# naver/dust3r

Hardware: NVIDIA H100
Metric: image-pairs/sec (512x384, ViT-L/B+DPT) (higher is better)
Workload: dtype bf16

## Files before the change

dust3r_b200/_lib.py:

```python
from __future__ import annotations

import ctypes as C
import os

from ._lib_fwd import Model

_HERE = os.path.dirname(os.path.abspath(__file__))
LIB_PATH = os.path.join(_HERE, 'libdust3r_b200.so')

_lib = None


class D3RError(RuntimeError):
    pass


class AlignDesc(C.Structure):
    _fields_ = [
        ('n_imgs', C.c_int32), ('n_edges', C.c_int32), ('n_entries', C.c_int32), ('n_chunks', C.c_int32),
        ('max_deg', C.c_int32), ('max_chunks', C.c_int32), ('chunk_px', C.c_int32), ('dist_l2', C.c_int32), ('norm_pw_scale', C.c_int32),
        ('tied_focal', C.c_int32), ('eval_only', C.c_int32),
        ('base_scale', C.c_float), ('pw_break', C.c_float), ('focal_break', C.c_float), ('adam_eps', C.c_float),
        ('beta1', C.c_float), ('beta2', C.c_float),
        ('img_hw', C.c_void_p), ('img_pix_off', C.c_void_p), ('img_ent_ptr', C.c_void_p),
# ... 44 lines not shown
    'd3r_align_small_step': (i32, [_DESC, i32, vp]),
    'd3r_align_reduce_block': (i32, [i32, i32, C.POINTER(i64), C.POINTER(i64)]),
    'd3r_align_loss_grad': (i32, [_DESC, vp, vp, vp, vp]),
    'd3r_align_overflow_flag': (i32, [_DESC, C.POINTER(i32), vp]),
    'd3r_align_pts3d': (i32, [_DESC, vp, vp]),
    'd3r_align_set_debug': (i32, [vp]),
    'd3r_sizeof_pack_entry': (i32, []),
    'd3r_align_stream_slots_per_item': (i32, []),
    'd3r_align_stream_warps_per_cta': (i32, []),
    'd3r_align_stream_max_window': (i32, []),
    'd3r_align_pack_entries': (i32, [vp, i32, i32, i32, i32, vp, vp]),
    'd3r_gemm_bf16': (i32, [vp, vp, vp, vp, vp, vp, i32, i32, i32, i64, u32, vp, vp, i32, i32, i32, vp]),
    'd3r_conv3x3_bf16': (i32, [vp, vp, vp, vp, vp, vp, vp, i32, i32, i32, i32, i32, u32, vp]),
    'd3r_attention_hd64': (i32, [vp, i64, vp, i64, vp, i64, vp, i64, i32, i32, i32, i32, f32, vp]),
    'd3r_conv_transpose_bf16': (i32, [vp, vp, vp, vp, i32, i32, i32, i32, i32, i32, vp]),
    'd3r_conv3x3_head_tail': (i32, [vp, vp, vp, vp, vp, vp, vp, i32, i32, i32, i32, i32, f32, f32, vp]),
    'd3r_layernorm_bf16': (i32, [vp, vp, vp, vp, i32, i32, f32, vp]),
    'd3r_upsample2x_bf16': (i32, [vp, vp, i32, i32, i32, i32, i32, i32, vp]),
    'd3r_im2col_3x3_s2_bf16': (i32, [vp, vp, i32, i32, i32, i32, vp]),
    'd3r_patch_im2col16': (i32, [vp, vp, i32, i32, i32, vp]),
    'd3r_linear_head_postprocess': (i32, [vp, vp, vp, i32, i32, i32, i32, i32, i32, f32, f32, vp]),
    'd3r_set_gemm_impl': (None, [i32]),
    'd3r_set_gemm_store': (None, [i32]),
    'd3r_set_conv_store': (None, [i32]),
    'd3r_set_attention_impl': (None, [i32]),
    'd3r_clean_pointcloud': (i32, [i32, vp, vp, i32, vp, vp, vp, vp, vp, f32, f32, vp]),
    'd3r_procrustes_moments': (i32, [i32, i32, vp, vp, vp, vp, vp]),
    'd3r_weiszfeld_focal': (i32, [i32, i32, i32, vp, vp, i32, vp, vp]),
    'd3r_nearest_neighbours': (i32, [i32, i32, vp, vp, vp, vp]),
    'd3r_image_resize_crop_normalize': (i32, [vp, i32, i32, i32, i32, vp, vp, i32, vp, vp, i32, i32, i32, i32, i32, i32, i32,
                                              vp, vp, vp, vp]),
    'd3r_sizeof_jpeg_desc': (i32, []),
    'd3r_jpeg_decode_workspace_bytes': (i64, [_JPEG, i64]),
    'd3r_jpeg_decode': (i32, [_JPEG, vp, i64, vp, vp, vp, i64, vp]),
    'd3r_segment_sky_workspace_bytes': (i64, [i32, i64]),
    'd3r_segment_sky': (i32, [i32, vp, vp, i32, i64, vp, vp, vp, i64, vp]),
    'd3r_nanmedian_workspace_bytes': (i64, [i32]),
    'd3r_segmented_nanmedian': (i32, [i32, i64, vp, vp, vp, i64, vp]),
    'd3r_criterion_workspace_bytes': (i64, [i32, i64, i64, i32]),
    'd3r_criterion': (i32, [i32, i64, i64, i32, i32, f32, f32] + [vp] * 15 + [i64, vp]),
    'd3r_sizeof_model': (i32, []),
    'd3r_encode_workspace_bytes': (i64, [_MODEL, i32, i32, i32]),
    'd3r_encode_images': (i32, [_MODEL, vp, i32, i32, i32, vp, vp, i64, vp]),
    'd3r_decode_workspace_bytes': (i64, [_MODEL, i32, i32, i32, i32, i32]),
    'd3r_decode_pairs': (i32, [_MODEL, vp, i32, i32, i32, vp, i32, i32, i32, C.POINTER(i32), C.POINTER(i32), i32,
                               vp, vp, vp, vp, vp, i64, vp]),
# ... 80 lines not shown
```

dust3r_b200/csrc/gemm_host.cu:

```cuda
#include "gemm_wgmma.cuh"
#include "gemm_host.h"
#include "prof.h"

namespace d3r {
namespace gemm {

static int pick_block_n(int N, int mode, uint32_t flags, int conv_m_tiles = 0) {
  if (flags & F_HEAD_FINAL) return 128;
  if (conv_m_tiles > 0) return (N == 256 && (conv_m_tiles + 1) / 2 >= 4 * (num_sms() / 2)) ? 256 : 128;
  if (N % 256 == 0 && pick_epi(mode, flags) != EPI_GENERIC) return 256;
  if (N % 128 == 0) return 128;
  if (N % 64 == 0) return 64;
  return (N > 128) ? 128 : 64;
}

static int g_impl = 2;
constexpr int kPairMinKb = 4;
static bool use_pair(int bn, int num_kb) { return bn >= 128 && (g_impl == 1 || (g_impl == 2 && num_kb >= kPairMinKb)); }

static int g_store = 1;
static int g_conv_store = 1;

static int grid_for(bool pair, int m_tiles, int n_tiles) {
  if (pair) {
    const int items = ((m_tiles + 1) / 2) * n_tiles;
    const int max_clusters = num_sms() / 2;
    return 2 * (items < max_clusters ? items : max_clusters);
  }
  const int items = m_tiles * n_tiles;
  return items < num_sms() ? items : num_sms();
}

static const char* prof_tag(const Params& p, int bn, bool pair) {
  return (p.mode == 1) ? ((p.flags & F_HEAD_FINAL) ? (pair ? "conv3x3_head_tail_2cta" : "conv3x3_head_tail")
                                                   : (pair ? "conv3x3_wgmma_2cta" : "conv3x3_wgmma"))
                       : (bn == 256 ? (pair ? "gemm_wgmma_2cta_bn256" : "gemm_wgmma_bn256")
                                    : (pair ? "gemm_wgmma_2cta_bn128" : (bn == 128 ? "gemm_wgmma_bn128" : "gemm_wgmma_bn64")));
}

template <int BN, int EPI, bool PAIR, bool TMA_STORE = false>
static int launch(const CUtensorMap& ta, const CUtensorMap& tb, const CUtensorMap& to, const Params& p, int m_tiles, int n_tiles,
                  cudaStream_t st) {
  constexpr int kSmem = Cfg<BN, TMA_STORE>::kSmemBytes;
  static unsigned long long attr_devices = 0;
  if (first_launch_on_this_device(attr_devices))
    D3R_CUDA(cudaFuncSetAttribute(gemm_kernel<BN, EPI, PAIR, TMA_STORE>, cudaFuncAttributeMaxDynamicSharedMemorySize, kSmem));
  const int grid = grid_for(PAIR, m_tiles, n_tiles);
  char detail[96];
  snprintf(detail, sizeof(detail), "M=%d N=%d K=%d flags=0x%x mode=%d epi=%d", p.M, p.N, p.K, (unsigned)p.flags, p.mode, EPI);
  prof::Scope scope(prof_tag(p, BN, PAIR), st, 2.0 * double(p.M) * double(p.N) * double(p.K), 0.0, 1, detail);
  D3R_CUDA(pdl::launch_clustered(gemm_kernel<BN, EPI, PAIR, TMA_STORE>, dim3(grid), dim3(kNumThreads), size_t(kSmem), st, PAIR ? 2 : 1,
                                 ta, tb, to, p));
  D3R_LAUNCH_CHECK();
  return D3R_OK;
}

template <int BN, bool PAIR>
static int launch_conv(const CUtensorMap& ta, const CUtensorMap& tb, const CUtensorMap& to, const ConvMaps& cm, const Params& p,
                       int m_tiles, int n_tiles, cudaStream_t st) {
  constexpr int kSmem = Cfg<BN, true>::kSmemBytes;
  static unsigned long long attr_devices = 0;
  if (first_launch_on_this_device(attr_devices))
    D3R_CUDA(cudaFuncSetAttribute(conv_kernel<BN, PAIR>, cudaFuncAttributeMaxDynamicSharedMemorySize, kSmem));
  const int grid = grid_for(PAIR, m_tiles, n_tiles);
  char detail[96];
  snprintf(detail, sizeof(detail), "M=%d N=%d K=%d flags=0x%x mode=%d epi=%d", p.M, p.N, p.K, (unsigned)p.flags, p.mode, EPI_GENERIC);
  prof::Scope scope(prof_tag(p, BN, PAIR), st, 2.0 * double(p.M) * double(p.N) * double(p.K), 0.0, 1, detail);
  D3R_CUDA(pdl::launch_clustered(conv_kernel<BN, PAIR>, dim3(grid), dim3(kNumThreads), size_t(kSmem), st, PAIR ? 2 : 1, ta, tb, to, cm, p));
  D3R_LAUNCH_CHECK();
  return D3R_OK;
}

template <int BN, bool PAIR>
static int dispatch_epi(int epi, const CUtensorMap& ta, const CUtensorMap& tb, const CUtensorMap* to, const Params& p, int m_tiles,
                        int n_tiles, cudaStream_t st) {
  if constexpr (BN == 256) {
    if (to) {
      switch (epi) {
        case EPI_RESID: return launch<BN, EPI_RESID, PAIR, true>(ta, tb, *to, p, m_tiles, n_tiles, st);
        case EPI_ACT: return launch<BN, EPI_ACT, PAIR, true>(ta, tb, *to, p, m_tiles, n_tiles, st);
        case EPI_ROPE: return launch<BN, EPI_ROPE, PAIR, true>(ta, tb, *to, p, m_tiles, n_tiles, st);
      }
    }
  }
  switch (epi) {
    case EPI_RESID: return launch<BN, EPI_RESID, PAIR>(ta, tb, tb, p, m_tiles, n_tiles, st);
    case EPI_ACT: return launch<BN, EPI_ACT, PAIR>(ta, tb, tb, p, m_tiles, n_tiles, st);
// ... 13 lines not shown
    case 256: return pair ? dispatch_epi<256, true>(epi, ta, tb, to, p, m_tiles, n_tiles, st) : dispatch_epi<256, false>(epi, ta, tb, to, p, m_tiles, n_tiles, st);
    case 128: return pair ? dispatch_epi<128, true>(epi, ta, tb, nullptr, p, m_tiles, n_tiles, st) : dispatch_epi<128, false>(epi, ta, tb, nullptr, p, m_tiles, n_tiles, st);
    case 64: return launch<64, EPI_GENERIC, false>(ta, tb, tb, p, m_tiles, n_tiles, st);
  }
  set_error("unsupported BLOCK_N %d", bn);
  return D3R_ERR_INVALID;
}

static int make_tmap_b(CUtensorMap* m, const void* B, int N, int taps, int Kc, int bn, int num_kb, const char* op) {
  cuuint64_t dims[3] = {(cuuint64_t)Kc, (cuuint64_t)taps, (cuuint64_t)N};
  cuuint64_t str[2] = {(cuuint64_t)Kc * 2, (cuuint64_t)taps * Kc * 2};
  cuuint32_t box[3] = {(cuuint32_t)BLOCK_K, 1, (cuuint32_t)(use_pair(bn, num_kb) ? bn / 2 : bn)};
  return encode_tensor_map(m, B, 3, dims, str, box, op);
}

int gemm_bf16(const void* A, long long lda, const void* B, Params p, cudaStream_t st) {
  D3R_CHECK_ARG(A && B, "gemm: null operand");
  D3R_CHECK_ARG(p.M > 0 && p.N > 0 && p.K > 0, "gemm: bad shape %d %d %d", p.M, p.N, p.K);
  D3R_CHECK_ARG(p.N % 32 == 0, "gemm: N=%d must be a multiple of 32", p.N);
  D3R_CHECK_ARG(p.K % 8 == 0 && lda % 8 == 0, "gemm: K=%d / lda=%lld must be multiples of 8 (16-byte TMA strides)", p.K, lda);
  D3R_CHECK_ARG((reinterpret_cast<uintptr_t>(A) & 15) == 0 && (reinterpret_cast<uintptr_t>(B) & 15) == 0, "gemm: operands must be 16-byte aligned");
  p.mode = 0;
  p.num_kb = (p.K + BLOCK_K - 1) / BLOCK_K;
  const int bn = pick_block_n(p.N, p.mode, p.flags);
  CUtensorMap ta, tb;
  {
    cuuint64_t dims[2] = {(cuuint64_t)p.K, (cuuint64_t)p.M};
    cuuint64_t str[1] = {(cuuint64_t)lda * 2};
    cuuint32_t box[2] = {(cuuint32_t)BLOCK_K, (cuuint32_t)BLOCK_M};
    int rc = encode_tensor_map(&ta, A, 2, dims, str, box, "gemm");
    if (rc) return rc;
  }
  int rc = make_tmap_b(&tb, B, p.N, 1, p.K, bn, p.num_kb, "gemm");
  if (rc) return rc;
  CUtensorMap to;
  const bool f32 = (p.flags & F_RESID_INPLACE) != 0;
  const long long row_bytes = p.ldo * (f32 ? 4 : 2);
  const bool staged = g_store == 1 && bn == 256 && pick_epi(p.mode, p.flags) != EPI_GENERIC && p.ldo >= p.N && row_bytes % 16 == 0 &&
                      (reinterpret_cast<uintptr_t>(p.out) & 15) == 0;
  if (staged) {
    cuuint64_t dims[2] = {(cuuint64_t)p.N, (cuuint64_t)p.M};
    cuuint64_t str[1] = {(cuuint64_t)row_bytes};
    cuuint32_t box[2] = {(cuuint32_t)(f32 ? 32 : 64), 64};
    rc = encode_tensor_map(&to, p.out, 2, dims, str, box, "gemm output", f32 ? CU_TENSOR_MAP_DATA_TYPE_FLOAT32 : CU_TENSOR_MAP_DATA_TYPE_BFLOAT16);
    if (rc) return rc;
  }
  return dispatch(bn, ta, tb, staged ? &to : nullptr, p, (p.M + BLOCK_M - 1) / BLOCK_M, st);
}

static int make_tmap_conv_io(CUtensorMap* m, const void* base, int B, int H, int W, int C, int tile_w, const char* op) {
  const int bw = tile_w < 64 ? tile_w : 64;
  cuuint64_t dims[4] = {(cuuint64_t)C, (cuuint64_t)W, (cuuint64_t)H, (cuuint64_t)B};
  cuuint64_t str[3] = {(cuuint64_t)C * 2, (cuuint64_t)W * C * 2, (cuuint64_t)H * W * C * 2};
  cuuint32_t box[4] = {64, (cuuint32_t)bw, (cuuint32_t)(64 / bw), 1};
  return encode_tensor_map(m, base, 4, dims, str, box, op);
}

static bool aligned16(const void* ptr) { return (reinterpret_cast<uintptr_t>(ptr) & 15) == 0; }

int conv3x3_bf16(const void* x_nhwc, const void* w_packed, int B, int H, int W, int Cin, int Cout, Params p, cudaStream_t st) {
  D3R_CHECK_ARG(x_nhwc && w_packed, "conv3x3: null operand");
  D3R_CHECK_ARG(Cin % 8 == 0 && Cout % 32 == 0, "conv3x3: Cin=%d must be a multiple of 8 and Cout=%d of 32", Cin, Cout);
  p.mode = 1;
  p.M = B * H * W;
  p.N = Cout;
  p.cin_blocks = (Cin + BLOCK_K - 1) / BLOCK_K;
  p.K = 9 * Cin;
  p.num_kb = 9 * p.cin_blocks;
  p.cB = B; p.cH = H; p.cW = W;
  int tw = 16;
// ... 57 lines not shown
                      float* conf, int B, int H, int W, int depth_mode, int conf_mode, float conf_min, float conf_max, cudaStream_t st) {
  D3R_CHECK_ARG(x_nhwc && w_packed && w4 && b4 && pts3d, "conv3x3_head_tail: null buffer");
  D3R_CHECK_ARG(B > 0 && H > 0 && W > 0, "conv3x3_head_tail: bad shape B=%d H=%d W=%d", B, H, W);
  D3R_CHECK_ARG(depth_mode >= 0 && depth_mode <= 2, "conv3x3_head_tail: depth_mode %d out of range", depth_mode);
  D3R_CHECK_ARG(conf_mode >= 0 && conf_mode <= 2, "conv3x3_head_tail: conf_mode %d out of range", conf_mode);
  D3R_CHECK_ARG(conf_mode == 0 || conf, "conv3x3_head_tail: conf_mode %d without a conf buffer", conf_mode);
  Params p{};
  p.flags = F_HEAD_FINAL | (bias ? F_BIAS : 0);
  p.bias = bias;
  p.w4 = w4; p.b4 = b4;
  p.pts3d = pts3d; p.conf = conf;
  p.depth_mode = depth_mode; p.conf_mode = conf_mode;
  p.conf_min = conf_min; p.conf_max = conf_max;
  return conv3x3_bf16(x_nhwc, w_packed, B, H, W, 128, 128, p, st);
}

}
}

using namespace d3r;

extern "C" void d3r_set_gemm_impl(int32_t impl) { gemm::g_impl = impl; }
extern "C" void d3r_set_gemm_store(int32_t store) { gemm::g_store = store; }
extern "C" void d3r_set_conv_store(int32_t store) { gemm::g_conv_store = store; }

extern "C" int d3r_gemm_bf16(const void* A, const void* B, void* out, const float* bias, const void* add0, void* out2,
                             int32_t M, int32_t N, int32_t K, int64_t ldo, uint32_t flags, const float* rope_cos,
                             const float* rope_sin, int32_t rope_cols, int32_t tokens_per_img, int32_t grid_w, void* stream) {
  gemm::Params p{};
  p.M = M; p.N = N; p.K = K;
  p.flags = flags;
  p.out = out; p.out2 = out2; p.add0 = add0; p.bias = bias; p.ldo = ldo;
  p.rope_cos = rope_cos; p.rope_sin = rope_sin; p.rope_cols = rope_cols; p.tokens_per_img = tokens_per_img; p.grid_w = grid_w;
  D3R_CHECK_ARG(!(flags & gemm::F_BIAS) || bias, "gemm: F_BIAS without bias");
  D3R_CHECK_ARG(!(flags & gemm::F_ROPE) || (rope_cos && rope_sin && tokens_per_img > 0 && grid_w > 0), "gemm: F_ROPE without tables");
  D3R_CHECK_ARG(!(flags & (gemm::F_CONVT | gemm::F_HEAD_FINAL)),
                "gemm: F_CONVT / F_HEAD_FINAL have their own entry points, d3r_conv_transpose_bf16 / d3r_conv3x3_head_tail");
  return gemm::gemm_bf16(A, K, B, p, (cudaStream_t)stream);
}

extern "C" int d3r_conv3x3_bf16(const void* x_nhwc, const void* w_packed, void* out, const float* bias, const void* add0,
                                const void* add1, void* out2, int32_t B, int32_t H, int32_t W, int32_t Cin, int32_t Cout,
                                uint32_t flags, void* stream) {
  gemm::Params p{};
  p.flags = flags;
  p.out = out; p.out2 = out2; p.add0 = add0; p.add1 = add1; p.bias = bias;
// ... 16 lines not shown
```

dust3r_b200/csrc/gemm_wgmma.cuh:

```cuda
#pragma once
#include "d3r_common.cuh"
#include "sm90_ptx.cuh"
#include "pdl.cuh"

namespace d3r {
namespace gemm {

constexpr int BLOCK_M = 128;
constexpr int BLOCK_K = 64;
constexpr int WGMMA_K = 16;
constexpr int kNumThreads = 384;
constexpr int kConsumerWarps = 8;

enum : uint32_t {
  F_BIAS = 1u << 0,
  F_GELU = 1u << 1,
  F_RELU = 1u << 2,
  F_OUT_F32 = 1u << 3,
  F_RESID_INPLACE = 1u << 4,
  F_ADD0 = 1u << 5,
  F_ADD1 = 1u << 6,
  F_OUT2_RELU = 1u << 7,
  F_ROPE = 1u << 8,
  F_CONVT = 1u << 9,
// ... 4 lines not shown
struct Params {
  int M, N, K;
  int num_kb;
  int mode;
  uint32_t flags;
  void* out;
  void* out2;
  const void* add0;
  const void* add1;
  const float* bias;
  long long ldo;
  const float* rope_cos;
  const float* rope_sin;
  int rope_cols, tokens_per_img, grid_w;
  int cB, cH, cW, cin_blocks, tile_w, tile_h, tiles_x, tiles_y;
  int tk, th_in, tw_in, tCout;
  const float* w4;
  const float* b4;
  float* pts3d;
  float* conf;
  int depth_mode;
  int conf_mode;
  float conf_min, conf_max;
};

enum : int { EPI_GENERIC = 0, EPI_RESID = 1, EPI_ACT = 2, EPI_ROPE = 3, EPI_CONV = 4 };
template <int EPI> struct EpiMask { static constexpr uint32_t value = 0xFFFFFFFFu; };
template <> struct EpiMask<EPI_RESID> { static constexpr uint32_t value = F_BIAS | F_RESID_INPLACE; };
template <> struct EpiMask<EPI_ACT> { static constexpr uint32_t value = F_BIAS | F_GELU | F_RELU; };
template <> struct EpiMask<EPI_ROPE> { static constexpr uint32_t value = F_BIAS | F_ROPE; };
template <> struct EpiMask<EPI_CONV> { static constexpr uint32_t value = F_BIAS | F_RELU | F_ADD0 | F_ADD1 | F_OUT2_RELU; };

struct ConvMaps {
  CUtensorMap out2, add0, add1;
};

__host__ __device__ inline int pick_epi(int mode, uint32_t flags) {
  if (mode != 0) return EPI_GENERIC;
  if ((flags & ~F_BIAS) == F_RESID_INPLACE) return EPI_RESID;
  if ((flags & ~EpiMask<EPI_ACT>::value) == 0) return EPI_ACT;
  if ((flags & ~EpiMask<EPI_ROPE>::value) == 0) return EPI_ROPE;
  return EPI_GENERIC;
}

template <int BLOCK_N, bool TMA_STORE = false>
struct Cfg {
  static constexpr int kStageA = BLOCK_M * BLOCK_K * 2;
  static constexpr int kStageB = BLOCK_N * BLOCK_K * 2;
  static constexpr int kStages = (BLOCK_N == 256) ? 4 : (BLOCK_N == 128) ? 6 : 8;
  static constexpr int kRing = kStages * (kStageA + kStageB);
  static constexpr int kOutBuf = 64 * 128;
  static constexpr int kStaging = TMA_STORE ? 2 * 2 * kOutBuf : 0;
  static constexpr int kSmemBytes = kRing + kStaging + 1024  + 256  + (TMA_STORE ? 0 : (4 * 128 + 16) * 4) ;
  static_assert(kSmemBytes <= 227 * 1024, "shared memory of one CTA");
};

__device__ __forceinline__ float gelu_erf(float x) {
  constexpr float kU = 0.84932180028801904f;
  constexpr float kP = 0.3275911f * 0.70710678118654752f / kU;
  const float u = fabsf(x) * kU;
  const float t = ptx::rcp_approx(fmaf(kP, u, 1.f));
  float poly = fmaf(0.5f * 1.061405429f, t, 0.5f * -1.453152027f);
  poly = fmaf(poly, t, 0.5f * 1.421413741f);
  poly = fmaf(poly, t, 0.5f * -0.284496736f);
  poly = fmaf(poly, t, 0.5f * 0.254829592f);
  const float e = ptx::ex2_approx(-u * u);
  const float h = x * (poly * t * e);
  return fmaxf(x, 0.f) - fabsf(h);
}

template <int BLOCK_N, int EPI, bool PAIR, bool TMA_STORE>
__device__ __forceinline__ void gemm_body(const CUtensorMap& tmap_a, const CUtensorMap& tmap_b, const CUtensorMap& tmap_o,
                                          const ConvMaps* cm, const Params& p) {
  static_assert(EPI == EPI_CONV ? (TMA_STORE && (BLOCK_N == 256 || BLOCK_N == 128))
                                : (!TMA_STORE || (BLOCK_N == 256 && EPI != EPI_GENERIC)),
                "TMA-store epilogue: specialised projection epilogues on 128x256 tiles, the conv epilogue on 128x256 / 128x128");
  using C = Cfg<BLOCK_N, TMA_STORE>;
  extern __shared__ uint8_t smem_raw[];
  uint8_t* smem = reinterpret_cast<uint8_t*>((reinterpret_cast<uintptr_t>(smem_raw) + 1023) & ~uintptr_t(1023));
  uint8_t* smem_a = smem;
  uint8_t* smem_b = smem + C::kStages * C::kStageA;
  uint8_t* smem_o = smem + C::kRing;
  uint64_t* bars = reinterpret_cast<uint64_t*>(smem + C::kRing + C::kStaging);
  uint64_t* full_bar = bars;
  uint64_t* empty_bar = bars + C::kStages;
  uint64_t* add_bar = bars + 2 * C::kStages;
  float* s_w4 = reinterpret_cast<float*>(reinterpret_cast<uint8_t*>(bars) + 256);

  const int warp = threadIdx.x >> 5, lane = threadIdx.x & 31;
  const uint32_t rank = PAIR ? ptx::cluster_ctarank() : 0u;
  const int n_tiles = (p.N + BLOCK_N - 1) / BLOCK_N;
  const int m_tiles = (p.mode == 1) ? p.cB * p.tiles_y * p.tiles_x : (p.M + BLOCK_M - 1) / BLOCK_M;
  const int m_groups = PAIR ? (m_tiles + 1) / 2 : m_tiles;
  const int total_items = m_groups * n_tiles;
  const int first_item = PAIR ? blockIdx.x / 2 : blockIdx.x;
  const int item_stride = PAIR ? gridDim.x / 2 : gridDim.x;

  if (threadIdx.x == 0) {
    ptx::prefetch_tmap(&tmap_a);
    ptx::prefetch_tmap(&tmap_b);
    if constexpr (TMA_STORE) ptx::prefetch_tmap(&tmap_o);
    for (int s = 0; s < C::kStages; ++s) {
      ptx::mbar_init(ptx::smem_u32(&full_bar[s]), 1);
      ptx::mbar_init(ptx::smem_u32(&empty_bar[s]), (PAIR ? 2 : 1) * kConsumerWarps);
    }
    if constexpr (EPI == EPI_CONV) {
      ptx::prefetch_tmap(&cm->out2);
      ptx::prefetch_tmap(&cm->add0);
      ptx::prefetch_tmap(&cm->add1);
      ptx::mbar_init(ptx::smem_u32(&add_bar[0]), 1);
      ptx::mbar_init(ptx::smem_u32(&add_bar[1]), 1);
    }
    ptx::fence_barrier_init();
  }
  if (!TMA_STORE && (p.flags & F_HEAD_FINAL) && threadIdx.x >= 128) {
    for (int i = threadIdx.x - 128; i < 4 * 128 + 4; i += 256) s_w4[i] = (i < 512) ? p.w4[i] : p.b4[i - 512];
  }
  __syncthreads();
  if constexpr (PAIR) ptx::cluster_sync();
  pdl::sync_with_predecessor();

  if (warp < 4) {
    ptx::setmaxnreg_dec<40>();
    if (warp == 0 && ptx::elect_one()) {
      int stage = 0;
      uint32_t phase = 0;
      for (int item = first_item; item < total_items; item += item_stride) {
        const int tn = item % n_tiles, tm = (item / n_tiles) * (PAIR ? 2 : 1) + int(rank);
        int cb = 0, cy0 = 0, cx0 = 0;
        if (p.mode == 1) {
          cb = tm / (p.tiles_y * p.tiles_x);
          const int r = tm - cb * (p.tiles_y * p.tiles_x);
          cy0 = (r / p.tiles_x) * p.tile_h;
          cx0 = (r % p.tiles_x) * p.tile_w;
        }
        for (int kb = 0; kb < p.num_kb; ++kb) {
          ptx::mbar_wait(ptx::smem_u32(&empty_bar[stage]), phase ^ 1);
          const uint32_t fb = ptx::smem_u32(&full_bar[stage]);
          ptx::mbar_arrive_expect_tx(fb, C::kStageA + C::kStageB);
          const uint32_t sa = ptx::smem_u32(smem_a + stage * C::kStageA);
          const uint32_t sb = ptx::smem_u32(smem_b + stage * C::kStageB);
          int ka, kt = 0;
          if (p.mode == 1) {
            const int tap = kb / p.cin_blocks, cblk = kb - tap * p.cin_blocks;
            const int dy = tap / 3, dx = tap - dy * 3;
            ptx::tma_load_4d(sa, &tmap_a, fb, cblk * BLOCK_K, cx0 + dx - 1, cy0 + dy - 1, cb);
            ka = cblk * BLOCK_K;
            kt = tap;
          } else {
            ptx::tma_load_2d(sa, &tmap_a, fb, kb * BLOCK_K, tm * BLOCK_M);
            ka = kb * BLOCK_K;
          }
          if constexpr (PAIR) {
            constexpr int kHalf = BLOCK_N / 2;
            ptx::tma_load_3d_mc(sb + rank * (kHalf * BLOCK_K * 2), &tmap_b, fb, ka, kt, tn * BLOCK_N + int(rank) * kHalf, 0x3);
          } else {
            ptx::tma_load_3d(sb, &tmap_b, fb, ka, kt, tn * BLOCK_N);
          }
          if (++stage == C::kStages) { stage = 0; phase ^= 1; }
        }
      }
    }
  } else {
    ptx::setmaxnreg_inc<232>();
    const int wg = (threadIdx.x >> 7) - 1;
    const int wq = warp & 3;
    const int q = lane & 3;
    const uint32_t flags = p.flags & EpiMask<EPI>::value;
    constexpr int kNB = BLOCK_N / 8;
    float acc[BLOCK_N / 2];
    int stage = 0;
    uint32_t phase = 0;
    uint32_t out_chunk = 0;
    auto release = [&](int s) {
      if (lane == 0) {
        if constexpr (PAIR) {
          ptx::mbar_arrive_cluster(ptx::smem_u32(&empty_bar[s]), 0);
          ptx::mbar_arrive_cluster(ptx::smem_u32(&empty_bar[s]), 1);
        } else {
          ptx::mbar_arrive(ptx::smem_u32(&empty_bar[s]));
        }
      }
    };
    const bool conv_issuer = EPI == EPI_CONV && (threadIdx.x & 127) == 0;
    const bool conv_two = EPI == EPI_CONV && (flags & (F_OUT2_RELU | F_ADD1)) != 0;
    const bool conv_add = EPI == EPI_CONV && (flags & (F_ADD0 | F_ADD1)) != 0;
    uint32_t add_phase = 0;
    auto conv_box = [&](int tm, int& bx, int& by, int& bb) {
// ... 12 lines not shown
      const uint32_t bar = ptx::smem_u32(&add_bar[wg]);
      ptx::mbar_arrive_expect_tx(bar, uint32_t(C::kOutBuf) * (((flags & F_ADD0) ? 1u : 0u) + ((flags & F_ADD1) ? 1u : 0u)));
      if (flags & F_ADD0) ptx::tma_load_4d(b0, &cm->add0, bar, ch, bx, by, bb);
      if (flags & F_ADD1) ptx::tma_load_4d(out_buf(1), &cm->add1, bar, ch, bx, by, bb);
    };
    for (int item = first_item; item < total_items; item += item_stride) {
      const int tn = item % n_tiles, tm = (item / n_tiles) * (PAIR ? 2 : 1) + int(rank);
      if constexpr (EPI == EPI_CONV) {
        if (conv_add && conv_issuer) issue_addends(tm, tn * BLOCK_N);
      }
      int prev = -1;
      for (int kb = 0; kb < p.num_kb; ++kb) {
        ptx::mbar_wait(ptx::smem_u32(&full_bar[stage]), phase);
        const uint64_t da = ptx::desc_kmajor_sw128(ptx::smem_u32(smem_a + stage * C::kStageA + wg * 64 * 128));
        const uint64_t db = ptx::desc_kmajor_sw128(ptx::smem_u32(smem_b + stage * C::kStageB));
        ptx::wgmma_fence();
#pragma unroll
        for (int k = 0; k < BLOCK_K / WGMMA_K; ++k) {
          if constexpr (BLOCK_N == 256) ptx::wgmma_m64n256k16_ss(acc, da + uint64_t(2 * k), db + uint64_t(2 * k), (kb | k) != 0 ? 1u : 0u);
          else if constexpr (BLOCK_N == 128) ptx::wgmma_m64n128k16_ss(acc, da + uint64_t(2 * k), db + uint64_t(2 * k), (kb | k) != 0 ? 1u : 0u);
          else ptx::wgmma_m64n64k16_ss(acc, da + uint64_t(2 * k), db + uint64_t(2 * k), (kb | k) != 0 ? 1u : 0u);
        }
        ptx::wgmma_commit();
        ptx::wgmma_wait<1>();
        if (prev >= 0) release(prev);
        prev = stage;
        if (++stage == C::kStages) { stage = 0; phase ^= 1; }
      }
      ptx::wgmma_wait<0>();
      ptx::reg_fence(acc);
      release(prev);

      bool valid[2];
      long long row_off[2];
      int tok[2] = {0, 0};
      long long pix[2] = {0, 0};
      int ct_b[2] = {0, 0}, ct_iy[2] = {0, 0}, ct_ix[2] = {0, 0};
#pragma unroll
      for (int h = 0; h < 2; ++h) {
        const int row_in_tile = wg * 64 + wq * 16 + (lane >> 2) + 8 * h;
        if (p.mode == 1) {
          const int cb = tm / (p.tiles_y * p.tiles_x);
          const int r = tm - cb * (p.tiles_y * p.tiles_x);
          const int y = (r / p.tiles_x) * p.tile_h + row_in_tile / p.tile_w;
          const int x = (r % p.tiles_x) * p.tile_w + row_in_tile % p.tile_w;
          valid[h] = (tm < m_tiles) && (y < p.cH) && (x < p.cW);
          pix[h] = (long long)(cb * p.cH + y) * p.cW + x;
          row_off[h] = pix[h] * p.ldo;
        } else {
          const int row = tm * BLOCK_M + row_in_tile;
          valid[h] = row < p.M;
          row_off[h] = (long long)row * p.ldo;
          if (flags & F_ROPE) tok[h] = row % p.tokens_per_img;
          if (flags & F_CONVT) {
// ... 83 lines not shown
            }
          ptx::fence_proxy_async();
          if (!conv_add && !conv_two && conv_issuer) ptx::bulk_wait_group_read<0>();
          ptx::named_bar_sync(1 + wg, 128);
          const int ch = tn * BLOCK_N + c * 64;
          if (conv_issuer) {
            ptx::tma_store_4d(&tmap_o, b0, ch, bx, by, bb);
            if (flags & F_OUT2_RELU) ptx::tma_store_4d(&cm->out2, b1, ch, bx, by, bb);
            ptx::bulk_commit_group();
          }
          ++out_chunk;
          if (conv_add && conv_issuer && c + 1 < BLOCK_N / 64) issue_addends(tm, ch + 64);
        }
        continue;
      }
      if constexpr (TMA_STORE) {
        constexpr bool kF32 = (EPI == EPI_RESID);
        constexpr int kChunkCols = kF32 ? 32 : 64;
        constexpr int kChunkNB = kChunkCols / 8;
        const bool issuer = (threadIdx.x & 127) == 0;
        const uint32_t sw = lane >> 2;
#pragma unroll
        for (int c = 0; c < BLOCK_N / kChunkCols; ++c) {
          const uint32_t buf = ptx::smem_u32(smem_o + (wg * 2 + (out_chunk & 1)) * C::kOutBuf);
#pragma unroll
          for (int j = 0; j < kChunkNB; ++j)
#pragma unroll
            for (int h = 0; h < 2; ++h) {
              const uint32_t row = wq * 16 + (lane >> 2) + 8 * h;
              float v0 = acc[4 * (c * kChunkNB + j) + 2 * h], v1 = acc[4 * (c * kChunkNB + j) + 2 * h + 1];
              if (flags & F_RELU) { v0 = fmaxf(v0, 0.f); v1 = fmaxf(v1, 0.f); }
              if constexpr (kF32) {
                ptx::st_shared_v2_f32(buf + row * 128 + (((2 * j + (q >> 1)) ^ sw) << 4) + (q & 1) * 8, v0, v1);
              } else {
                ptx::st_shared_b32(buf + row * 128 + ((j ^ sw) << 4) + q * 4, pack_bf16x2(v0, v1));
              }
            }
          ptx::fence_proxy_async();
          if (issuer) ptx::bulk_wait_group_read<0>();
          ptx::named_bar_sync(1 + wg, 128);
          if (issuer) {
            const int c0 = tn * BLOCK_N + c * kChunkCols, r0 = tm * BLOCK_M + wg * 64;
            if constexpr (kF32) ptx::tma_reduce_add_2d(&tmap_o, buf, c0, r0);
            else ptx::tma_store_2d(&tmap_o, buf, c0, r0);
            ptx::bulk_commit_group();
          }
          ++out_chunk;
        }
        continue;
      }
      if (flags & F_HEAD_FINAL) {
        float head_acc[2][4] = {{0.f, 0.f, 0.f, 0.f}, {0.f, 0.f, 0.f, 0.f}};
#pragma unroll
        for (int j = 0; j < kNB; ++j)
#pragma unroll
          for (int h = 0; h < 2; ++h)
#pragma unroll
            for (int e = 0; e < 2; ++e) {
              const float r = fmaxf(acc[4 * j + 2 * h + e], 0.f);
              const int c = 8 * j + 2 * q + e;
#pragma unroll
              for (int o = 0; o < 4; ++o) head_acc[h][o] += r * s_w4[o * 128 + c];
// ... 49 lines not shown
            if (flags & F_OUT2_BF16) *reinterpret_cast<uint32_t*>(reinterpret_cast<__nv_bfloat16*>(p.out2) + off) = pack_bf16x2(v0, v1);
          } else {
            *reinterpret_cast<uint32_t*>(reinterpret_cast<__nv_bfloat16*>(p.out) + off) = pack_bf16x2(v0, v1);
            if (flags & F_OUT2_RELU)
              *reinterpret_cast<uint32_t*>(reinterpret_cast<__nv_bfloat16*>(p.out2) + off) = pack_bf16x2(fmaxf(v0, 0.f), fmaxf(v1, 0.f));
          }
        }
      }
    }
    if constexpr (TMA_STORE) {
      if ((threadIdx.x & 127) == 0) ptx::bulk_wait_group<0>();
    }
  }
  if constexpr (PAIR) ptx::cluster_sync();
}

template <int BLOCK_N, int EPI, bool PAIR, bool TMA_STORE>
__global__ void __launch_bounds__(kNumThreads, 1)
gemm_kernel(const __grid_constant__ CUtensorMap tmap_a, const __grid_constant__ CUtensorMap tmap_b,
            const __grid_constant__ CUtensorMap tmap_o, const Params p) {
  gemm_body<BLOCK_N, EPI, PAIR, TMA_STORE>(tmap_a, tmap_b, tmap_o, nullptr, p);
}

template <int BLOCK_N, bool PAIR>
__global__ void __launch_bounds__(kNumThreads, 1)
conv_kernel(const __grid_constant__ CUtensorMap tmap_a, const __grid_constant__ CUtensorMap tmap_b,
            const __grid_constant__ CUtensorMap tmap_o, const __grid_constant__ ConvMaps cm, const Params p) {
  gemm_body<BLOCK_N, EPI_CONV, PAIR, true>(tmap_a, tmap_b, tmap_o, &cm, p);
}

}
}
```

dust3r_b200/csrc/sm90_ptx.cuh:

```cuda
#pragma once
#include <cuda.h>
#include <cuda_runtime.h>
#include <cuda_bf16.h>
#include <cstdint>

namespace d3r {
namespace ptx {

__device__ __forceinline__ uint32_t smem_u32(const void* p) { return static_cast<uint32_t>(__cvta_generic_to_shared(p)); }

__device__ __forceinline__ bool elect_one() {
  uint32_t pred = 0;
  asm volatile(
      "{\n"
      ".reg .b32 %%rx;\n"
      ".reg .pred %%px;\n"
      "elect.sync %%rx|%%px, %1;\n"
      "@%%px mov.s32 %0, 1;\n"
      "}\n"
      : "+r"(pred)
      : "r"(0xffffffffu));
  return pred != 0;
}

// ... 83 lines not shown
}
__device__ __forceinline__ void tma_store_4d(const void* tmap, uint32_t src, int c0, int c1, int c2, int c3) {
  asm volatile("cp.async.bulk.tensor.4d.global.shared::cta.tile.bulk_group [%0, {%2, %3, %4, %5}], [%1];"
               ::"l"(reinterpret_cast<uint64_t>(tmap)), "r"(src), "r"(c0), "r"(c1), "r"(c2), "r"(c3) : "memory");
}
__device__ __forceinline__ void tma_reduce_add_2d(const void* tmap, uint32_t src, int c0, int c1) {
  asm volatile("cp.reduce.async.bulk.tensor.2d.global.shared::cta.add.tile.bulk_group [%0, {%2, %3}], [%1];"
               ::"l"(reinterpret_cast<uint64_t>(tmap)), "r"(src), "r"(c0), "r"(c1) : "memory");
}
__device__ __forceinline__ void bulk_commit_group() { asm volatile("cp.async.bulk.commit_group;" ::: "memory"); }
template <int N> __device__ __forceinline__ void bulk_wait_group_read() { asm volatile("cp.async.bulk.wait_group.read %0;" ::"n"(N) : "memory"); }
template <int N> __device__ __forceinline__ void bulk_wait_group() { asm volatile("cp.async.bulk.wait_group %0;" ::"n"(N) : "memory"); }
__device__ __forceinline__ void st_shared_b32(uint32_t addr, uint32_t v) { asm volatile("st.shared.b32 [%0], %1;" ::"r"(addr), "r"(v) : "memory"); }
__device__ __forceinline__ uint32_t ld_shared_b32(uint32_t addr) {
  uint32_t v;
  asm volatile("ld.shared.b32 %0, [%1];" : "=r"(v) : "r"(addr) : "memory");
  return v;
}
__device__ __forceinline__ void st_shared_v2_f32(uint32_t addr, float a, float b) {
  asm volatile("st.shared.v2.f32 [%0], {%1, %2};" ::"r"(addr), "f"(a), "f"(b) : "memory");
}
__device__ __forceinline__ void named_bar_sync(uint32_t id, uint32_t count) { asm volatile("bar.sync %0, %1;" ::"r"(id), "r"(count) : "memory"); }

__device__ __forceinline__ uint32_t cluster_ctarank() {
  uint32_t r;
  asm volatile("mov.u32 %0, %%cluster_ctarank;" : "=r"(r));
  return r;
}
__device__ __forceinline__ void cluster_sync() {
  asm volatile("barrier.cluster.arrive.release.aligned;\nbarrier.cluster.wait.acquire.aligned;" ::: "memory");
}
__device__ __forceinline__ void mbar_arrive_cluster(uint32_t bar, uint32_t rank) {
  asm volatile(
      "{\n"
      ".reg .b32 raddr;\n"
      "mapa.shared::cluster.u32 raddr, %0, %1;\n"
      "mbarrier.arrive.shared::cluster.b64 _, [raddr];\n"
      "}\n" ::"r"(bar), "r"(rank) : "memory");
}

__device__ __forceinline__ float ex2_approx(float x) { float y; asm("ex2.approx.ftz.f32 %0, %1;" : "=f"(y) : "f"(x)); return y; }
__device__ __forceinline__ float rcp_approx(float x) { float y; asm("rcp.approx.ftz.f32 %0, %1;" : "=f"(y) : "f"(x)); return y; }
__device__ __forceinline__ float rsqrt_approx(float x) { float y; asm("rsqrt.approx.ftz.f32 %0, %1;" : "=f"(y) : "f"(x)); return y; }
__device__ __forceinline__ float sqrt_approx(float x) { float y; asm("sqrt.approx.ftz.f32 %0, %1;" : "=f"(y) : "f"(x)); return y; }

template <int N> __device__ __forceinline__ void setmaxnreg_dec() { asm volatile("setmaxnreg.dec.sync.aligned.u32 %0;" ::"n"(N)); }
// ... 80 lines not shown
```

include/dust3r_b200.h:

```cpp
#ifndef DUST3R_B200_H_
#define DUST3R_B200_H_

#include <stddef.h>
#include <stdint.h>

#ifdef __cplusplus
extern "C" {
#endif

#define D3R_OK 0
#define D3R_ERR_INVALID (-1)
#define D3R_ERR_CUDA (-2)
#define D3R_ERR_UNSUPPORTED_DEVICE (-3)

const char* d3r_last_error(void);
int d3r_abi_version(void);
int d3r_check_device(void);

long long d3r_launch_count(void);
void d3r_launch_count_reset(void);
void d3r_prof_enable(int on);
int d3r_prof_report(char* buf, int cap);
int d3r_prof_dump(char* buf, int cap);

// ... 122 lines not shown

int d3r_conv_transpose_bf16(const void* x_nhwc_dev, const void* w_packed_dev, void* out_dev, const float* bias_dev, int32_t B,
                            int32_t h, int32_t w, int32_t Cin, int32_t Cout, int32_t k, void* stream);

int d3r_conv3x3_head_tail(const void* x_nhwc_dev, const void* w_packed_dev, const float* bias_dev, const float* w4_dev,
                          const float* b4_dev, float* pts3d_dev, float* conf_dev, int32_t B, int32_t H, int32_t W, int32_t depth_mode,
                          int32_t conf_mode, float conf_min, float conf_max, void* stream);

int d3r_layernorm_bf16(const float* x_dev, const float* g_dev, const float* b_dev, void* out_dev, int32_t M, int32_t C, float eps,
                       void* stream);

int d3r_upsample2x_bf16(const void* x_dev, void* out_dev, int32_t B, int32_t H, int32_t W, int32_t C, int32_t Ho, int32_t Wo,
                        void* stream);

int d3r_im2col_3x3_s2_bf16(const void* x_dev, void* out_dev, int32_t B, int32_t H, int32_t W, int32_t C, void* stream);

int d3r_patch_im2col16(const float* img_dev, void* out_dev, int32_t B, int32_t H, int32_t W, void* stream);

int d3r_linear_head_postprocess(const float* feat_dev, float* pts3d_dev, float* conf_dev, int32_t B, int32_t gh, int32_t gw,
                                int32_t nch, int32_t depth_mode, int32_t conf_mode, float conf_min, float conf_max, void* stream);

void d3r_set_gemm_impl(int32_t impl);
void d3r_set_gemm_store(int32_t store);
void d3r_set_conv_store(int32_t store);

void d3r_set_attention_impl(int32_t impl);

int d3r_clean_pointcloud(int32_t n_imgs, const int32_t* hw_dev, const int64_t* off_dev, int32_t max_area, const float* pts3d_dev,
                         float* conf_dev, const float* depth_dev, const float* K_dev, const float* cams_dev, float tol,
                         float bad_conf, void* stream);
int d3r_procrustes_moments(int32_t n_problems, int32_t n_points, const float* x_dev, const float* y_dev, const float* w_dev,
                           double* out_dev, void* stream);
int d3r_weiszfeld_focal(int32_t n_maps, int32_t H, int32_t W, const float* pts3d_dev, const float* pp_dev, int32_t steps,
                        float* focal_dev, void* stream);
int d3r_nearest_neighbours(int32_t n_queries, int32_t n_points, const float* queries_dev, const float* points_dev, int32_t* nn_dev,
                           void* stream);
int d3r_image_resize_crop_normalize(const uint8_t* src_dev, int32_t H0, int32_t W0, int32_t H1, int32_t W1,
                                    const int32_t* xbounds_dev, const int32_t* xcoefs_dev, int32_t kx,
                                    const int32_t* ybounds_dev, const int32_t* ycoefs_dev, int32_t ky, int32_t row0, int32_t rows,
                                    int32_t crop_x0, int32_t crop_y0, int32_t H2, int32_t W2, const float* lut_dev, uint8_t* tmp_dev,
                                    float* out_dev, void* stream);
typedef struct d3r_jpeg_huff {
  int32_t maxcode[18];
  int32_t valoff[18];
  uint16_t look[512];
  uint8_t val[256];
// ... 113 lines not shown
```

Measured before the change: 232.8.

## Add two-CTAs-per-SM 128x128 GEMM path for activation epilogue

Adds a gemm_kernel_2persm variant with 128x128 tiles, 288 threads, 3 stages, a single output staging buffer and no register reallocation, sized so two CTAs co-reside on one SM. It becomes the default (g_store=2) for paired, TMA-stored, activation-epilogue GEMMs whose N is a multiple of 256, such as the MLP fc1. The aim is to overlap one CTA's epilogue with the other's mainloop. Grid sizing now uses occupancy queries instead of the SM count. The cost is a shallower pipeline, wgmma_wait<0> each k-block, smaller tiles and tighter registers, which may lower mainloop throughput.

```diff
diff --git a/dust3r_b200/_lib.py b/dust3r_b200/_lib.py
--- a/dust3r_b200/_lib.py
+++ b/dust3r_b200/_lib.py
@@ -90,6 +90,8 @@
     'd3r_linear_head_postprocess': (i32, [vp, vp, vp, i32, i32, i32, i32, i32, i32, f32, f32, vp]),
     'd3r_set_gemm_impl': (None, [i32]),
     'd3r_set_gemm_store': (None, [i32]),
+    'd3r_gemm_2persm_occupancy': (i32, [C.POINTER(i32), C.POINTER(i32)]),
+    'd3r_gemm_record_smid': (None, [vp]),
     'd3r_set_conv_store': (None, [i32]),
     'd3r_set_attention_impl': (None, [i32]),
     'd3r_clean_pointcloud': (i32, [i32, vp, vp, i32, vp, vp, vp, vp, vp, f32, f32, vp]),
diff --git a/dust3r_b200/csrc/gemm_host.cu b/dust3r_b200/csrc/gemm_host.cu
--- a/dust3r_b200/csrc/gemm_host.cu
+++ b/dust3r_b200/csrc/gemm_host.cu
@@ -18,17 +18,51 @@
 constexpr int kPairMinKb = 4;
 static bool use_pair(int bn, int num_kb) { return bn >= 128 && (g_impl == 1 || (g_impl == 2 && num_kb >= kPairMinKb)); }
 
-static int g_store = 1;
+static int g_store = 2;
+static int* g_cta_smid = nullptr;
+
+static bool use_2persm(int N, int epi, bool pair) {
+  return g_store == 2 && pair && epi == EPI_ACT && N % 256 == 0;
+}
 static int g_conv_store = 1;
 
-static int grid_for(bool pair, int m_tiles, int n_tiles) {
+template <typename Kernel>
+static int resident_ctas(Kernel kernel, int threads, int smem, bool pair, int (&cache)[64]) {
+  int dev = 0;
+  cudaGetDevice(&dev);
+  int& n = cache[dev & 63];
+  if (n > 0) return n;
+  if (pair) {
+    cudaLaunchConfig_t cfg = {};
+    cfg.gridDim = dim3(2 * num_sms());
+    cfg.blockDim = dim3(threads);
+    cfg.dynamicSmemBytes = smem;
+    cudaLaunchAttribute at;
+    at.id = cudaLaunchAttributeClusterDimension;
+    at.val.clusterDim.x = 2;
+    at.val.clusterDim.y = 1;
+    at.val.clusterDim.z = 1;
+    cfg.attrs = &at;
+    cfg.numAttrs = 1;
+    int clusters = 0;
+    if (cudaOccupancyMaxActiveClusters(&clusters, kernel, &cfg) != cudaSuccess) clusters = 0;
+    n = 2 * clusters;
+  } else {
+    int per_sm = 0;
+    if (cudaOccupancyMaxActiveBlocksPerMultiprocessor(&per_sm, kernel, threads, smem) != cudaSuccess) per_sm = 0;
+    n = per_sm * num_sms();
+  }
+  return n;
+}
+
+static int grid_for(bool pair, int slots, int m_tiles, int n_tiles) {
   if (pair) {
     const int items = ((m_tiles + 1) / 2) * n_tiles;
-    const int max_clusters = num_sms() / 2;
+    const int max_clusters = slots / 2;
     return 2 * (items < max_clusters ? items : max_clusters);
   }
   const int items = m_tiles * n_tiles;
-  return items < num_sms() ? items : num_sms();
+  return items < slots ? items : slots;
 }
 
 static const char* prof_tag(const Params& p, int bn, bool pair) {
@@ -43,9 +77,11 @@
                   cudaStream_t st) {
   constexpr int kSmem = Cfg<BN, TMA_STORE>::kSmemBytes;
   static unsigned long long attr_devices = 0;
+  static int slots[64] = {};
   if (first_launch_on_this_device(attr_devices))
     D3R_CUDA(cudaFuncSetAttribute(gemm_kernel<BN, EPI, PAIR, TMA_STORE>, cudaFuncAttributeMaxDynamicSharedMemorySize, kSmem));
-  const int grid = grid_for(PAIR, m_tiles, n_tiles);
+  const int grid = grid_for(PAIR, resident_ctas(gemm_kernel<BN, EPI, PAIR, TMA_STORE>, kNumThreads, kSmem, PAIR, slots), m_tiles, n_tiles);
+  D3R_CHECK_ARG(grid > 0, "gemm: no CTA of gemm_kernel<%d, %d, %d, %d> fits on the device", BN, EPI, int(PAIR), int(TMA_STORE));
   char detail[96];
   snprintf(detail, sizeof(detail), "M=%d N=%d K=%d flags=0x%x mode=%d epi=%d", p.M, p.N, p.K, (unsigned)p.flags, p.mode, EPI);
   prof::Scope scope(prof_tag(p, BN, PAIR), st, 2.0 * double(p.M) * double(p.N) * double(p.K), 0.0, 1, detail);
@@ -55,14 +91,37 @@
   return D3R_OK;
 }
 
+template <int EPI>
+static int launch_2persm(const CUtensorMap& ta, const CUtensorMap& tb, const CUtensorMap& to, const Params& p, int m_tiles, int n_tiles,
+                         cudaStream_t st) {
+  using C = Cfg<128, true, 2>;
+  constexpr int kSmem = C::kSmemBytes;
+  static unsigned long long attr_devices = 0;
+  static int slots[64] = {};
+  if (first_launch_on_this_device(attr_devices))
+    D3R_CUDA(cudaFuncSetAttribute(gemm_kernel_2persm<EPI, true>, cudaFuncAttributeMaxDynamicSharedMemorySize, kSmem));
+  const int grid = grid_for(true, resident_ctas(gemm_kernel_2persm<EPI, true>, C::kThreads, kSmem, true, slots), m_tiles, n_tiles);
+  D3R_CHECK_ARG(grid > 0, "gemm: no CTA of gemm_kernel_2persm<%d> fits on the device", EPI);
+  Params pk = p;
+  pk.cta_smid = g_cta_smid;
+  char detail[96];
+  snprintf(detail, sizeof(detail), "M=%d N=%d K=%d flags=0x%x mode=%d epi=%d", p.M, p.N, p.K, (unsigned)p.flags, p.mode, EPI);
+  prof::Scope scope("gemm_wgmma_2cta_2persm_bn128", st, 2.0 * double(p.M) * double(p.N) * double(p.K), 0.0, 1, detail);
+  D3R_CUDA(pdl::launch_clustered(gemm_kernel_2persm<EPI, true>, dim3(grid), dim3(C::kThreads), size_t(kSmem), st, 2, ta, tb, to, pk));
+  D3R_LAUNCH_CHECK();
+  return D3R_OK;
+}
+
 template <int BN, bool PAIR>
 static int launch_conv(const CUtensorMap& ta, const CUtensorMap& tb, const CUtensorMap& to, const ConvMaps& cm, const Params& p,
                        int m_tiles, int n_tiles, cudaStream_t st) {
   constexpr int kSmem = Cfg<BN, true>::kSmemBytes;
   static unsigned long long attr_devices = 0;
+  static int slots[64] = {};
   if (first_launch_on_this_device(attr_devices))
     D3R_CUDA(cudaFuncSetAttribute(conv_kernel<BN, PAIR>, cudaFuncAttributeMaxDynamicSharedMemorySize, kSmem));
-  const int grid = grid_for(PAIR, m_tiles, n_tiles);
+  const int grid = grid_for(PAIR, resident_ctas(conv_kernel<BN, PAIR>, kNumThreads, kSmem, PAIR, slots), m_tiles, n_tiles);
+  D3R_CHECK_ARG(grid > 0, "conv3x3: no CTA of conv_kernel<%d, %d> fits on the device", BN, int(PAIR));
   char detail[96];
   snprintf(detail, sizeof(detail), "M=%d N=%d K=%d flags=0x%x mode=%d epi=%d", p.M, p.N, p.K, (unsigned)p.flags, p.mode, EPI_GENERIC);
   prof::Scope scope(prof_tag(p, BN, PAIR), st, 2.0 * double(p.M) * double(p.N) * double(p.K), 0.0, 1, detail);
@@ -122,7 +181,14 @@
   D3R_CHECK_ARG((reinterpret_cast<uintptr_t>(A) & 15) == 0 && (reinterpret_cast<uintptr_t>(B) & 15) == 0, "gemm: operands must be 16-byte aligned");
   p.mode = 0;
   p.num_kb = (p.K + BLOCK_K - 1) / BLOCK_K;
-  const int bn = pick_block_n(p.N, p.mode, p.flags);
+  const int epi = pick_epi(p.mode, p.flags);
+  int bn = pick_block_n(p.N, p.mode, p.flags);
+  const bool f32 = (p.flags & F_RESID_INPLACE) != 0;
+  const long long row_bytes = p.ldo * (f32 ? 4 : 2);
+  const bool tma_out = p.ldo >= p.N && row_bytes % 16 == 0 && (reinterpret_cast<uintptr_t>(p.out) & 15) == 0;
+  const bool two_per_sm = bn == 256 && tma_out && use_2persm(p.N, epi, use_pair(256, p.num_kb));
+  if (two_per_sm) bn = 128;
+  const bool staged = two_per_sm || (g_store >= 1 && bn == 256 && epi != EPI_GENERIC && tma_out);
   CUtensorMap ta, tb;
   {
     cuuint64_t dims[2] = {(cuuint64_t)p.K, (cuuint64_t)p.M};
@@ -134,10 +200,6 @@
   int rc = make_tmap_b(&tb, B, p.N, 1, p.K, bn, p.num_kb, "gemm");
   if (rc) return rc;
   CUtensorMap to;
-  const bool f32 = (p.flags & F_RESID_INPLACE) != 0;
-  const long long row_bytes = p.ldo * (f32 ? 4 : 2);
-  const bool staged = g_store == 1 && bn == 256 && pick_epi(p.mode, p.flags) != EPI_GENERIC && p.ldo >= p.N && row_bytes % 16 == 0 &&
-                      (reinterpret_cast<uintptr_t>(p.out) & 15) == 0;
   if (staged) {
     cuuint64_t dims[2] = {(cuuint64_t)p.N, (cuuint64_t)p.M};
     cuuint64_t str[1] = {(cuuint64_t)row_bytes};
@@ -145,7 +207,9 @@
     rc = encode_tensor_map(&to, p.out, 2, dims, str, box, "gemm output", f32 ? CU_TENSOR_MAP_DATA_TYPE_FLOAT32 : CU_TENSOR_MAP_DATA_TYPE_BFLOAT16);
     if (rc) return rc;
   }
-  return dispatch(bn, ta, tb, staged ? &to : nullptr, p, (p.M + BLOCK_M - 1) / BLOCK_M, st);
+  const int m_tiles = (p.M + BLOCK_M - 1) / BLOCK_M;
+  if (two_per_sm) return launch_2persm<EPI_ACT>(ta, tb, to, p, m_tiles, p.N / 128, st);
+  return dispatch(bn, ta, tb, staged ? &to : nullptr, p, m_tiles, st);
 }
 
 static int make_tmap_conv_io(CUtensorMap* m, const void* base, int B, int H, int W, int C, int tile_w, const char* op) {
@@ -249,6 +313,20 @@
 
 extern "C" void d3r_set_gemm_impl(int32_t impl) { gemm::g_impl = impl; }
 extern "C" void d3r_set_gemm_store(int32_t store) { gemm::g_store = store; }
+extern "C" void d3r_gemm_record_smid(int32_t* cta_smid_dev) { gemm::g_cta_smid = cta_smid_dev; }
+
+extern "C" int d3r_gemm_2persm_occupancy(int32_t* ctas_per_sm, int32_t* clusters) {
+  D3R_CHECK_ARG(ctas_per_sm && clusters, "d3r_gemm_2persm_occupancy: null output");
+  using C = gemm::Cfg<128, true, 2>;
+  const auto kernel = gemm::gemm_kernel_2persm<gemm::EPI_ACT, true>;
+  D3R_CUDA(cudaFuncSetAttribute(kernel, cudaFuncAttributeMaxDynamicSharedMemorySize, C::kSmemBytes));
+  int per_sm = 0;
+  D3R_CUDA(cudaOccupancyMaxActiveBlocksPerMultiprocessor(&per_sm, kernel, C::kThreads, C::kSmemBytes));
+  int slots[64] = {};
+  *ctas_per_sm = per_sm;
+  *clusters = gemm::resident_ctas(kernel, C::kThreads, C::kSmemBytes, true, slots) / 2;
+  return D3R_OK;
+}
 extern "C" void d3r_set_conv_store(int32_t store) { gemm::g_conv_store = store; }
 
 extern "C" int d3r_gemm_bf16(const void* A, const void* B, void* out, const float* bias, const void* add0, void* out2,
diff --git a/dust3r_b200/csrc/gemm_wgmma.cuh b/dust3r_b200/csrc/gemm_wgmma.cuh
--- a/dust3r_b200/csrc/gemm_wgmma.cuh
+++ b/dust3r_b200/csrc/gemm_wgmma.cuh
@@ -50,6 +50,7 @@
   int depth_mode;
   int conf_mode;
   float conf_min, conf_max;
+  int* cta_smid;
 };
 
 enum : int { EPI_GENERIC = 0, EPI_RESID = 1, EPI_ACT = 2, EPI_ROPE = 3, EPI_CONV = 4 };
@@ -71,16 +72,21 @@
   return EPI_GENERIC;
 }
 
-template <int BLOCK_N, bool TMA_STORE = false>
+template <int BLOCK_N, bool TMA_STORE = false, int CTAS_PER_SM = 1>
 struct Cfg {
+  static_assert(CTAS_PER_SM == 1 || (CTAS_PER_SM == 2 && BLOCK_N == 128 && TMA_STORE), "two CTAs per SM: 128x128, TMA store");
+  static constexpr int kThreads = (CTAS_PER_SM == 2) ? 288 : kNumThreads;
   static constexpr int kStageA = BLOCK_M * BLOCK_K * 2;
   static constexpr int kStageB = BLOCK_N * BLOCK_K * 2;
-  static constexpr int kStages = (BLOCK_N == 256) ? 4 : (BLOCK_N == 128) ? 6 : 8;
+  static constexpr int kStages = (CTAS_PER_SM == 2) ? 3 : (BLOCK_N == 256) ? 4 : (BLOCK_N == 128) ? 6 : 8;
   static constexpr int kRing = kStages * (kStageA + kStageB);
   static constexpr int kOutBuf = 64 * 128;
-  static constexpr int kStaging = TMA_STORE ? 2 * 2 * kOutBuf : 0;
-  static constexpr int kSmemBytes = kRing + kStaging + 1024  + 256  + (TMA_STORE ? 0 : (4 * 128 + 16) * 4) ;
+  static constexpr int kOutBufs = (CTAS_PER_SM == 2) ? 1 : 2;
+  static constexpr int kStaging = TMA_STORE ? 2 * kOutBufs * kOutBuf : 0;
+  static constexpr int kAlignSlack = (CTAS_PER_SM == 2) ? 0 : 1024;
+  static constexpr int kSmemBytes = kRing + kStaging + kAlignSlack + 256  + (TMA_STORE ? 0 : (4 * 128 + 16) * 4) ;
   static_assert(kSmemBytes <= 227 * 1024, "shared memory of one CTA");
+  static_assert(CTAS_PER_SM * (kSmemBytes + 1024) <= 228 * 1024, "shared memory of the CTAs of one SM, 1 KB reserved per CTA");
 };
 
 __device__ __forceinline__ float gelu_erf(float x) {
@@ -97,15 +103,17 @@
   return fmaxf(x, 0.f) - fabsf(h);
 }
 
-template <int BLOCK_N, int EPI, bool PAIR, bool TMA_STORE>
+template <int BLOCK_N, int EPI, bool PAIR, bool TMA_STORE, int CTAS_PER_SM = 1>
 __device__ __forceinline__ void gemm_body(const CUtensorMap& tmap_a, const CUtensorMap& tmap_b, const CUtensorMap& tmap_o,
                                           const ConvMaps* cm, const Params& p) {
-  static_assert(EPI == EPI_CONV ? (TMA_STORE && (BLOCK_N == 256 || BLOCK_N == 128))
-                                : (!TMA_STORE || (BLOCK_N == 256 && EPI != EPI_GENERIC)),
-                "TMA-store epilogue: specialised projection epilogues on 128x256 tiles, the conv epilogue on 128x256 / 128x128");
-  using C = Cfg<BLOCK_N, TMA_STORE>;
-  extern __shared__ uint8_t smem_raw[];
-  uint8_t* smem = reinterpret_cast<uint8_t*>((reinterpret_cast<uintptr_t>(smem_raw) + 1023) & ~uintptr_t(1023));
+  static_assert(EPI == EPI_CONV ? (TMA_STORE && (BLOCK_N == 256 || BLOCK_N == 128) && CTAS_PER_SM == 1)
+                                : (!TMA_STORE || (BLOCK_N == (CTAS_PER_SM == 2 ? 128 : 256) && EPI != EPI_GENERIC)),
+                "TMA-store epilogue: specialised projection epilogues on 128x256 tiles (128x128 with two CTAs per SM), the conv "
+                "epilogue on 128x256 / 128x128");
+  using C = Cfg<BLOCK_N, TMA_STORE, CTAS_PER_SM>;
+  extern __shared__ __align__(1024) uint8_t smem_raw[];
+  uint8_t* smem = C::kAlignSlack ? reinterpret_cast<uint8_t*>((reinterpret_cast<uintptr_t>(smem_raw) + 1023) & ~uintptr_t(1023))
+                                 : smem_raw;
   uint8_t* smem_a = smem;
   uint8_t* smem_b = smem + C::kStages * C::kStageA;
   uint8_t* smem_o = smem + C::kRing;
@@ -148,9 +156,10 @@
   if constexpr (PAIR) ptx::cluster_sync();
   pdl::sync_with_predecessor();
 
-  if (warp < 4) {
-    ptx::setmaxnreg_dec<40>();
-    if (warp == 0 && ptx::elect_one()) {
+  constexpr int kProducerWarp = (CTAS_PER_SM == 2) ? 8 : 0;
+  if (CTAS_PER_SM == 2 ? warp == kProducerWarp : warp < 4) {
+    if constexpr (CTAS_PER_SM == 1) ptx::setmaxnreg_dec<40>();
+    if (warp == kProducerWarp && ptx::elect_one()) {
       int stage = 0;
       uint32_t phase = 0;
       for (int item = first_item; item < total_items; item += item_stride) {
@@ -190,8 +199,8 @@
       }
     }
   } else {
-    ptx::setmaxnreg_inc<232>();
-    const int wg = (threadIdx.x >> 7) - 1;
+    if constexpr (CTAS_PER_SM == 1) ptx::setmaxnreg_inc<232>();
+    const int wg = (threadIdx.x >> 7) - (CTAS_PER_SM == 2 ? 0 : 1);
     const int wq = warp & 3;
     const int q = lane & 3;
     const uint32_t flags = p.flags & EpiMask<EPI>::value;
@@ -250,14 +259,19 @@
           else ptx::wgmma_m64n64k16_ss(acc, da + uint64_t(2 * k), db + uint64_t(2 * k), (kb | k) != 0 ? 1u : 0u);
         }
         ptx::wgmma_commit();
-        ptx::wgmma_wait<1>();
-        if (prev >= 0) release(prev);
-        prev = stage;
+        if constexpr (CTAS_PER_SM == 2) {
+          ptx::wgmma_wait<0>();
+          release(stage);
+        } else {
+          ptx::wgmma_wait<1>();
+          if (prev >= 0) release(prev);
+          prev = stage;
+        }
         if (++stage == C::kStages) { stage = 0; phase ^= 1; }
       }
       ptx::wgmma_wait<0>();
       ptx::reg_fence(acc);
-      release(prev);
+      if (CTAS_PER_SM == 1) release(prev);
 
       bool valid[2];
       long long row_off[2];
@@ -387,7 +401,11 @@
         const uint32_t sw = lane >> 2;
 #pragma unroll
         for (int c = 0; c < BLOCK_N / kChunkCols; ++c) {
-          const uint32_t buf = ptx::smem_u32(smem_o + (wg * 2 + (out_chunk & 1)) * C::kOutBuf);
+          const uint32_t buf = ptx::smem_u32(smem_o + (wg * C::kOutBufs + (out_chunk % C::kOutBufs)) * C::kOutBuf);
+          if constexpr (C::kOutBufs == 1) {
+            if (issuer) ptx::bulk_wait_group_read<0>();
+            ptx::named_bar_sync(1 + wg, 128);
+          }
 #pragma unroll
           for (int j = 0; j < kChunkNB; ++j)
 #pragma unroll
@@ -402,7 +420,7 @@
               }
             }
           ptx::fence_proxy_async();
-          if (issuer) ptx::bulk_wait_group_read<0>();
+          if (C::kOutBufs == 2 && issuer) ptx::bulk_wait_group_read<0>();
           ptx::named_bar_sync(1 + wg, 128);
           if (issuer) {
             const int c0 = tn * BLOCK_N + c * kChunkCols, r0 = tm * BLOCK_M + wg * 64;
@@ -498,6 +516,14 @@
   gemm_body<BLOCK_N, EPI, PAIR, TMA_STORE>(tmap_a, tmap_b, tmap_o, nullptr, p);
 }
 
+template <int EPI, bool PAIR>
+__global__ void __launch_bounds__(Cfg<128, true, 2>::kThreads, 2)
+gemm_kernel_2persm(const __grid_constant__ CUtensorMap tmap_a, const __grid_constant__ CUtensorMap tmap_b,
+                   const __grid_constant__ CUtensorMap tmap_o, const Params p) {
+  if (p.cta_smid != nullptr && threadIdx.x == 0) p.cta_smid[blockIdx.x] = int(ptx::smid());
+  gemm_body<128, EPI, PAIR, true, 2>(tmap_a, tmap_b, tmap_o, nullptr, p);
+}
+
 template <int BLOCK_N, bool PAIR>
 __global__ void __launch_bounds__(kNumThreads, 1)
 conv_kernel(const __grid_constant__ CUtensorMap tmap_a, const __grid_constant__ CUtensorMap tmap_b,
diff --git a/dust3r_b200/csrc/sm90_ptx.cuh b/dust3r_b200/csrc/sm90_ptx.cuh
--- a/dust3r_b200/csrc/sm90_ptx.cuh
+++ b/dust3r_b200/csrc/sm90_ptx.cuh
@@ -129,6 +129,11 @@
 }
 __device__ __forceinline__ void named_bar_sync(uint32_t id, uint32_t count) { asm volatile("bar.sync %0, %1;" ::"r"(id), "r"(count) : "memory"); }
 
+__device__ __forceinline__ uint32_t smid() {
+  uint32_t r;
+  asm volatile("mov.u32 %0, %%smid;" : "=r"(r));
+  return r;
+}
 __device__ __forceinline__ uint32_t cluster_ctarank() {
   uint32_t r;
   asm volatile("mov.u32 %0, %%cluster_ctarank;" : "=r"(r));
diff --git a/include/dust3r_b200.h b/include/dust3r_b200.h
--- a/include/dust3r_b200.h
+++ b/include/dust3r_b200.h
@@ -168,6 +168,8 @@
 
 void d3r_set_gemm_impl(int32_t impl);
 void d3r_set_gemm_store(int32_t store);
+int d3r_gemm_2persm_occupancy(int32_t* ctas_per_sm, int32_t* clusters);
+void d3r_gemm_record_smid(int32_t* cta_smid_dev);
 void d3r_set_conv_store(int32_t store);
 
 void d3r_set_attention_impl(int32_t impl);
```

Measured after the change: 234.4, median of 6. Within noise of the previous version (+0.7%).
